# YooSungHyun/RNNTransducer

Measured on AMD Instinct MI355X. Metric: utterances/sec, higher is better.
Workload: dtype f32

## Files before the change

### rnntransducer_amd/csrc/gemm_hp.hip

```cpp
#include "common.hpp"

#include <stdlib.h>

namespace rnnt {
namespace {

typedef _Float16 f16x8 __attribute__((ext_vector_type(8)));
typedef __attribute__((address_space(3))) void lds_void;

constexpr int HP_BM = 256, HP_BN = 256, HP_BK = 32;
constexpr int HP_STAGE = (HP_BM + HP_BN) * 128;
constexpr int HP_RSRC = 0x00027000;

__device__ __forceinline__ float hp_scale_from_amax(unsigned amax_bits) {
  int eb = (int)((amax_bits >> 23) & 255u);
  if (eb == 0) return 1.0f;
  eb = eb < 15 ? 15 : eb;
  return __uint_as_float((unsigned)(268 - eb) << 23);
}
__device__ __forceinline__ float hp_inv_scale_from_amax(unsigned amax_bits) {
  int eb = (int)((amax_bits >> 23) & 255u);
  if (eb == 0) return 1.0f;
  eb = eb < 15 ? 15 : eb;
  return __uint_as_float((unsigned)(eb - 14) << 23);
}

__global__ void __launch_bounds__(256) hp_colmax_kernel(const float* __restrict__ x, long rows, int C, long ld, long rows_per_chunk,
                                                        unsigned* __restrict__ out) {
  const int c = blockIdx.x * 256 + threadIdx.x;
  if (c >= C) return;
  const long r0 = (long)blockIdx.y * rows_per_chunk, r1 = min(rows, r0 + rows_per_chunk);
  unsigned m = 0;
  for (long r = r0; r < r1; ++r) m = max(m, __float_as_uint(x[r * ld + c]) & 0x7fffffffu);
  if (m != 0) atomicMax(out + c, m);
}

__device__ __forceinline__ void hp_split8(const float (&x)[8], float scale, u32x4& hi, u32x4& lo) {
  f16x8 h, l;
#pragma unroll
  for (int e = 0; e < 8; ++e) {
    const float v = x[e] * scale;
    const _Float16 a = (_Float16)v;
    h[e] = a;
    l[e] = (_Float16)(v - (float)a);
  }
  hi = __builtin_bit_cast(u32x4, h);
  lo = __builtin_bit_cast(u32x4, l);
}

__global__ void __launch_bounds__(256) hp_split_kernel(const float* __restrict__ x, long rows, int K, long ld, unsigned* __restrict__ amax,
                                                       char* __restrict__ out, const int* __restrict__ rowidx) {
  const int Kp = (K + 31) & ~31, cpr = Kp >> 3;
  const int lane = threadIdx.x & 63;
  const bool vec = (ld & 3) == 0 && (reinterpret_cast<uintptr_t>(x) & 15) == 0;
  for (long ri = (long)blockIdx.x * 4 + (threadIdx.x >> 6); ri < rows; ri += (long)gridDim.x * 4) {
    const long r = rowidx ? (long)rowidx[ri] : ri;
    const float* row = x + r * ld;
    unsigned m = 0;
    for (int c = lane; c < cpr; c += 64) {
      const int k = 8 * c;
      if (vec && k + 7 < K) {
        const u32x4 a = *reinterpret_cast<const u32x4*>(row + k), b = *reinterpret_cast<const u32x4*>(row + k + 4);
#pragma unroll
        for (int e = 0; e < 4; ++e) m = max(m, max(a[e] & 0x7fffffffu, b[e] & 0x7fffffffu));
      } else {
#pragma unroll
        for (int e = 0; e < 8; ++e)
          if (k + e < K) m = max(m, __float_as_uint(row[k + e]) & 0x7fffffffu);
      }
    }
#pragma unroll
    for (int o = 32; o > 0; o >>= 1) m = max(m, (unsigned)__shfl_xor((int)m, o));
    if (lane == 0) amax[r] = m;
    const float scale = hp_scale_from_amax(m);
    for (int c = lane; c < cpr; c += 64) {
      const int k = 8 * c;
      float v[8];
      if (vec && k + 7 < K) {
        const f32x4 a = *reinterpret_cast<const f32x4*>(row + k), b = *reinterpret_cast<const f32x4*>(row + k + 4);
        v[0] = a[0]; v[1] = a[1]; v[2] = a[2]; v[3] = a[3]; v[4] = b[0]; v[5] = b[1]; v[6] = b[2]; v[7] = b[3];
      } else {
#pragma unroll
        for (int e = 0; e < 8; ++e) v[e] = (k + e < K) ? row[k + e] : 0.f;
      }
      u32x4 hi, lo;
      hp_split8(v, scale, hi, lo);
      char* dst = out + (r * (Kp >> 5) + (c >> 2)) * 128 + 16 * (c & 3);
      *reinterpret_cast<u32x4*>(dst) = hi;
      *reinterpret_cast<u32x4*>(dst + 64) = lo;
    }
  }
}

__global__ void __launch_bounds__(256) hp_split_t_kernel(const float* __restrict__ x, int R, int K, long ld, int Ksrc, int shift,
                                                         const unsigned* __restrict__ amax, char* __restrict__ out,
                                                         const int* __restrict__ kidx) {
  __shared__ float tile[32][257];
  const int kb = blockIdx.x, r0 = blockIdx.y * 256;
  const int tid = threadIdx.x;
  const bool vec = (ld & 3) == 0 && (reinterpret_cast<uintptr_t>(x) & 15) == 0;
#pragma unroll
  for (int q = 0; q < 8; ++q) {
    const int kk = 4 * q + (tid >> 6);
    const int kdst = kb * 32 + kk;
    const int ksrc = (kidx ? (kdst < K ? kidx[kdst] : 0) : kdst) + shift;
    const int c = 4 * (tid & 63);
    f32x4 v = {0.f, 0.f, 0.f, 0.f};
    if (kdst < K && ksrc >= 0 && ksrc < Ksrc) {
      const float* src = x + (long)ksrc * ld + r0 + c;
      if (vec && r0 + c + 3 < R) {
        v = *reinterpret_cast<const f32x4*>(src);
      } else {
#pragma unroll
        for (int e = 0; e < 4; ++e)
          if (r0 + c + e < R) v[e] = src[e];
      }
    }
#pragma unroll
    for (int e = 0; e < 4; ++e) tile[kk][c + e] = v[e];
  }
  __syncthreads();
  const int Kp32 = (K + 31) >> 5;
#pragma unroll
  for (int ps = 0; ps < 4; ++ps) {
    const int rl = (tid >> 2) + 64 * ps, ch = tid & 3;
    if (r0 + rl < R) {
      float v[8];
#pragma unroll
      for (int e = 0; e < 8; ++e) v[e] = tile[8 * ch + e][rl];
      u32x4 hi, lo;
      hp_split8(v, hp_scale_from_amax(amax[r0 + rl]), hi, lo);
      char* dst = out + ((long)(r0 + rl) * Kp32 + kb) * 128 + 16 * ch;
      *reinterpret_cast<u32x4*>(dst) = hi;
      *reinterpret_cast<u32x4*>(dst + 64) = lo;
    }
  }
}

__global__ void __launch_bounds__(256) hp_split_both_kernel(const float* __restrict__ x, int M, int C, long ld, const unsigned* __restrict__ rowmax,
                                                            const unsigned* __restrict__ colmax, char* __restrict__ out_rm, char* __restrict__ out_t,
                                                            const int* __restrict__ rowidx) {
  __shared__ float tile[32][257];
  const int kb = blockIdx.x, c0 = blockIdx.y * 256;
  const int tid = threadIdx.x;
  const int Cp = (C + 31) & ~31;
  const bool vec = (ld & 3) == 0 && (reinterpret_cast<uintptr_t>(x) & 15) == 0;
#pragma unroll
  for (int q = 0; q < 4; ++q) {
    const int row = 8 * q + (tid >> 5), col = 8 * (tid & 31);
    const int ri = kb * 32 + row, c = c0 + col;
    const int r = (rowidx && ri < M) ? rowidx[ri] : ri;
    float v[8] = {0.f, 0.f, 0.f, 0.f, 0.f, 0.f, 0.f, 0.f};
    if (ri < M && c < C) {
      const float* src = x + (long)r * ld + c;
      if (vec && c + 7 < C) {
        const f32x4 a = *reinterpret_cast<const f32x4*>(src), b = *reinterpret_cast<const f32x4*>(src + 4);
        v[0] = a[0]; v[1] = a[1]; v[2] = a[2]; v[3] = a[3]; v[4] = b[0]; v[5] = b[1]; v[6] = b[2]; v[7] = b[3];
      } else {
#pragma unroll
        for (int e = 0; e < 8; ++e)
          if (c + e < C) v[e] = src[e];
      }
    }
    if (ri < M && c < Cp) {
      u32x4 hi, lo;
      hp_split8(v, hp_scale_from_amax(rowmax[r]), hi, lo);
      char* dst = out_rm + ((long)r * (Cp >> 5) + (c >> 5)) * 128 + 16 * ((c >> 3) & 3);
      *reinterpret_cast<u32x4*>(dst) = hi;
      *reinterpret_cast<u32x4*>(dst + 64) = lo;
    }
#pragma unroll
    for (int e = 0; e < 8; ++e) tile[row][col + e] = v[e];
  }
  __syncthreads();
  const int Mp32 = (M + 31) >> 5;
#pragma unroll
  for (int ps = 0; ps < 4; ++ps) {
    const int rl = (tid >> 2) + 64 * ps, ch = tid & 3;
    if (c0 + rl < C) {
      float v[8];
#pragma unroll
      for (int e = 0; e < 8; ++e) v[e] = tile[8 * ch + e][rl];
      u32x4 hi, lo;
      hp_split8(v, hp_scale_from_amax(colmax[c0 + rl]), hi, lo);
      char* dst = out_t + ((long)(c0 + rl) * Mp32 + kb) * 128 + 16 * ch;
      *reinterpret_cast<u32x4*>(dst) = hi;
      *reinterpret_cast<u32x4*>(dst + 64) = lo;
    }
  }
}

struct HpGemmK {
  int M, N, nkt;
  const char* A; unsigned a_pitch, a_bytes;
  const char* B; unsigned b_pitch, b_bytes;
  const unsigned* a_amax; const unsigned* b_amax;
  float* C; int c_div; long c_so, c_si;
  const float* bias;
  unsigned flags;
  int splits, kt_per_split;
  float* slab;
  int tiles_m, tiles_n;
  int group_m;
  const int* a_rowidx;
  const int* c_rowidx;
};

// ... 153 lines not shown
  return n * tiles_m + m;
}

template <bool F16>
__global__ void __launch_bounds__(512, 1) gemm_hp_kernel(const HpGemmK p) {
  extern __shared__ __attribute__((aligned(16))) char lds[];
  int bid = hp_xcd_remap(blockIdx.x, p.tiles_m * p.tiles_n);
  if (p.group_m > 0) bid = hp_grouped_tile(bid, p.tiles_m, p.tiles_n, p.group_m);
  hp_tile256<F16>(p, bid, blockIdx.y, lds);
}

constexpr int HPQ_MAX = 4;
struct HpGemmQ {
  HpGemmK prob[HPQ_MAX];
  int unit_end[HPQ_MAX];
  int nprob;
  unsigned xcd_skip;
  unsigned* counter;
};

template <bool F16>
__global__ void __launch_bounds__(512, 1) gemm_hpq_kernel(const HpGemmQ q) {
  extern __shared__ __attribute__((aligned(16))) char lds[];
  unsigned xcc;
  asm volatile("s_getreg_b32 %0, hwreg(HW_REG_XCC_ID)" : "=s"(xcc));
  xcc &= 7u;
  if ((q.xcd_skip >> xcc) & 1u) return;
  const unsigned allow = ~q.xcd_skip & 0xffu;
  const int nq = __builtin_popcount(allow);
  const int mine = __builtin_popcount(allow & ((1u << xcc) - 1u));
  int* next = reinterpret_cast<int*>(lds + 2 * HP_STAGE);
  const int total = q.unit_end[q.nprob - 1];
  for (int hop = 0; hop < nq; ++hop) {
    const int qi = (mine + hop) % nq;
    const int lo = (int)((long)total * qi / nq), hi = (int)((long)total * (qi + 1) / nq);
    while (true) {
      if (threadIdx.x == 0) {
        const int got = lo + (int)atomicAdd(q.counter + qi, 1u);
        *next = got;
        if (got < hi) atomicAdd(q.counter + 8, 1u);
      }
      __syncthreads();
      const int u = __builtin_amdgcn_readfirstlane(*next);
      __syncthreads();
      if (u >= hi) break;
      int pi = 0;
      while (u >= q.unit_end[pi]) ++pi;
      const HpGemmK& p = q.prob[pi];
      const int local = u - (pi ? q.unit_end[pi - 1] : 0);
      const int tn = local % p.tiles_n, z = (local / p.tiles_n) % p.splits, tm = local / (p.tiles_n * p.splits);
      hp_tile256<F16>(p, tn * p.tiles_m + tm, z, lds);
    }
  }
}

__global__ void hpq_check_kernel(unsigned* counter, unsigned total, unsigned* status) {
  if (counter[8] != total) {
    counter[9] = 1u;
    if (status) __hip_atomic_store(status, 2u, __ATOMIC_RELAXED, __HIP_MEMORY_SCOPE_AGENT);
  }
}

__global__ void __launch_bounds__(256) hp_splitk_reduce_kernel(const HpGemmK p) {
  const long total = (long)p.M * p.N;
  for (long i = (long)blockIdx.x * 256 + threadIdx.x; i < total; i += (long)gridDim.x * 256) {
    const int m = (int)(i / p.N), n = (int)(i % p.N);
    float s = 0.f;
    for (int z = 0; z < p.splits; ++z) s += p.slab[(long)z * total + i];
    if (p.bias) s += p.bias[n];
    const int mo = p.c_rowidx ? p.c_rowidx[m] : m;
    const long off = (long)(mo / p.c_div) * p.c_so + (long)(mo % p.c_div) * p.c_si + n;
    if (p.flags & RNNT_GEMM_ACCUM) s += p.C[off];
    p.C[off] = s;
  }
}

}

size_t hp_plane_bytes(int64_t rows, int64_t K) { return (size_t)rows * (size_t)ceil_div(K, 32) * 128; }

int hp_colmax(const float* x, int64_t rows, int64_t C, int64_t ld, uint32_t* amax, hipStream_t s) {
  RNNT_CHECK_HIP(hipMemsetAsync(amax, 0, (size_t)C * 4, s));
  if (rows == 0 || C == 0) return RNNT_OK;
  long chunks = ceil_div(2048, ceil_div(C, 256));
  if (chunks > ceil_div(rows, 64)) chunks = ceil_div(rows, 64);
  if (chunks < 1) chunks = 1;
  const long rpc = ceil_div(rows, chunks);
  ProfScope prof(RNNT_K_HP_SPLIT, 4.0 * (double)rows * (double)C, s);
  hipLaunchKernelGGL(hp_colmax_kernel, dim3((unsigned)ceil_div(C, 256), (unsigned)ceil_div(rows, rpc)), dim3(256), 0, s, x, (long)rows, (int)C,
                     (long)ld, rpc, amax);
  RNNT_CHECK_LAUNCH();
  return RNNT_OK;
}

int hp_split(const float* x, int64_t rows, int64_t K, int64_t ld, uint32_t* amax, void* planes, hipStream_t s, const int* rowidx) {
  if (rows == 0) return RNNT_OK;
  const long blocks = ceil_div(rows, 4);
  ProfScope prof(RNNT_K_HP_SPLIT, 8.0 * (double)rows * (double)K, s);
  hipLaunchKernelGGL(hp_split_kernel, dim3((unsigned)(blocks < 8192 ? blocks : 8192)), dim3(256), 0, s, x, (long)rows, (int)K, (long)ld, amax,
                     (char*)planes, rowidx);
  RNNT_CHECK_LAUNCH();
  return RNNT_OK;
}

int hp_split_t(const float* x, int64_t R, int64_t K, int64_t ld, int64_t Ksrc, int64_t shift, const uint32_t* amax, void* planes,
               hipStream_t s, const int* kidx) {
  if (R == 0 || K == 0) return RNNT_OK;
  ProfScope prof(RNNT_K_HP_SPLIT, 8.0 * (double)R * (double)K, s);
  hipLaunchKernelGGL(hp_split_t_kernel, dim3((unsigned)ceil_div(K, 32), (unsigned)ceil_div(R, 256)), dim3(256), 0, s, x, (int)R, (int)K, (long)ld,
                     (int)Ksrc, (int)shift, amax, (char*)planes, kidx);
  RNNT_CHECK_LAUNCH();
  return RNNT_OK;
}

int hp_split_both(const float* x, int64_t M, int64_t C, int64_t ld, const uint32_t* rowmax, const uint32_t* colmax, void* planes_rm,
                  void* planes_t, hipStream_t s, const int* rowidx) {
  if (M == 0 || C == 0) return RNNT_OK;
  ProfScope prof(RNNT_K_HP_SPLIT, 12.0 * (double)M * (double)C, s);
  hipLaunchKernelGGL(hp_split_both_kernel, dim3((unsigned)ceil_div(M, 32), (unsigned)ceil_div(C, 256)), dim3(256), 0, s, x, (int)M, (int)C, (long)ld,
                     rowmax, colmax, (char*)planes_rm, (char*)planes_t, rowidx);
  RNNT_CHECK_LAUNCH();
  return RNNT_OK;
}

struct HpGemmPlan {
  int tiles_m, tiles_n, group_m, splits, kt_per_split;
  size_t workspace_bytes_wanted;
};
static HpGemmPlan hp_gemm_plan(int64_t M, int64_t N, int64_t K, size_t workspace_bytes) {
  HpGemmPlan pl;
  pl.tiles_m = (int)ceil_div(M, HP_BM); pl.tiles_n = (int)ceil_div(N, HP_BN);
  const long tiles = (long)pl.tiles_m * pl.tiles_n;
  const long nkt = ceil_div(K, HP_BK);
  {
    static const int env_gm = getenv("RNNT_GEMM_HP_GROUP_M") ? atoi(getenv("RNNT_GEMM_HP_GROUP_M")) : -1;
    pl.group_m = env_gm >= 0 ? env_gm : (tiles >= 256 ? 8 : 4);
  }
  long want = 1;
  if (tiles < 192 && nkt >= 64) {
    want = ceil_div(256, tiles);
    if (want > nkt / 32) want = nkt / 32;
    if (want > 32) want = 32;
    if (want < 2) want = 1;
  }
  const size_t slab = (size_t)M * (size_t)N * 4;
  pl.workspace_bytes_wanted = want >= 2 ? (size_t)want * slab : 0;
  const size_t by_ws = workspace_bytes / slab;
  long splits = (size_t)want > by_ws ? (long)by_ws : want;
  if (splits < 2) splits = 1;
  pl.kt_per_split = (int)ceil_div(nkt, splits);
  pl.splits = (int)ceil_div(nkt, pl.kt_per_split);
  return pl;
}

size_t hp_gemm_workspace_bytes(int64_t M, int64_t N, int64_t K) { return hp_gemm_plan(M, N, K, 0).workspace_bytes_wanted; }

int hp_gemm(const void* A, const uint32_t* a_amax, const void* B, const uint32_t* b_amax, int64_t M, int64_t N, int64_t K, float* C,
            int64_t c_div, int64_t c_so, int64_t c_si, const float* bias, unsigned flags, void* workspace, size_t workspace_bytes,
            hipStream_t s, const int* a_rowidx, int64_t a_plane_rows, const int* c_rowidx) {
  RNNT_CHECK_ARG(A && B && C && a_amax && b_amax, "gemm_hp: null operand");
  RNNT_CHECK_ARG(!a_rowidx || a_plane_rows >= M, "gemm_hp: a gathered A operand needs the row count of its planes");
  RNNT_CHECK_ARG(M >= 1 && N >= 1 && K >= 1 && M < (1ll << 31) && N < (1ll << 31) && K < (1ll << 31), "gemm_hp: bad dims");
  RNNT_CHECK_ARG(c_div >= 1, "gemm_hp: c_div must be >= 1");
  RNNT_CHECK_ARG(((reinterpret_cast<uintptr_t>(A) | reinterpret_cast<uintptr_t>(B)) & 127) == 0, "gemm_hp: planes must be 128-byte aligned");
  HpGemmK k;
  k.M = (int)M; k.N = (int)N; k.nkt = (int)ceil_div(K, HP_BK);
  const size_t ab = hp_plane_bytes(a_rowidx ? a_plane_rows : M, K), bb = hp_plane_bytes(N, K);
  RNNT_CHECK_ARG(ab < (1ull << 32) && bb < (1ull << 32), "gemm_hp: an operand exceeds the 4 GB a buffer resource addresses");
  k.A = (const char*)A; k.a_pitch = (unsigned)k.nkt * 128u; k.a_bytes = (unsigned)ab;
  k.B = (const char*)B; k.b_pitch = (unsigned)k.nkt * 128u; k.b_bytes = (unsigned)bb;
  k.a_amax = a_amax; k.b_amax = b_amax;
  k.C = C; k.c_div = (int)(c_div > 0x7fffffff ? 0x7fffffff : c_div); k.c_so = c_so; k.c_si = c_si;
  k.bias = bias; k.flags = flags;
  k.a_rowidx = a_rowidx; k.c_rowidx = c_rowidx;
  const bool f16 = (flags & RNNT_GEMM_HP_F16) != 0u;
  const HpGemmPlan pl = hp_gemm_plan(M, N, K, workspace ? workspace_bytes : 0);
  k.tiles_m = pl.tiles_m; k.tiles_n = pl.tiles_n; k.group_m = pl.group_m;
  k.splits = pl.splits; k.kt_per_split = pl.kt_per_split;
  const int tiles = k.tiles_m * k.tiles_n, splits = k.splits;
  k.slab = (float*)workspace;
  if (f16) RNNT_CHECK_HIP(hipFuncSetAttribute((const void*)gemm_hp_kernel<true>, hipFuncAttributeMaxDynamicSharedMemorySize, 2 * HP_STAGE));
  else RNNT_CHECK_HIP(hipFuncSetAttribute((const void*)gemm_hp_kernel<false>, hipFuncAttributeMaxDynamicSharedMemorySize, 2 * HP_STAGE));
  {
    ProfScope prof(RNNT_K_GEMM_HP, 2.0 * (double)M * (double)N * (double)K, s);
    if (f16) hipLaunchKernelGGL(gemm_hp_kernel<true>, dim3(tiles, splits), dim3(512), 2 * HP_STAGE, s, k);
    else hipLaunchKernelGGL(gemm_hp_kernel<false>, dim3(tiles, splits), dim3(512), 2 * HP_STAGE, s, k);
    RNNT_CHECK_LAUNCH();
    if (splits > 1) {
      const long blocks = ceil_div((long)M * N, 256);
      hipLaunchKernelGGL(hp_splitk_reduce_kernel, dim3((unsigned)(blocks < 2048 ? blocks : 2048)), dim3(256), 0, s, k);
      RNNT_CHECK_LAUNCH();
    }
  }
// ... 190 lines not shown
```

### rnntransducer_amd/csrc/lstm_layer.hip

```cpp
#include "lstm_shared.hpp"

#include <string.h>

namespace rnnt {
namespace {

__global__ void db_reduce_kernel(const float* __restrict__ part, int rows_per_dir, int H, int ngate, float* __restrict__ o0,
                                 float* __restrict__ o1, int accumulate, float* __restrict__ p0 = nullptr,
                                 float* __restrict__ p1 = nullptr) {
  const int c = blockIdx.x * 256 + threadIdx.x, d = blockIdx.y;
  if (c >= 4 * H || (c & 3) >= ngate) return;
  const float* src = part + (long)d * rows_per_dir * 4 * H + c;
  float s = 0.f;
  for (int r = 0; r < rows_per_dir; ++r) s += src[(long)r * 4 * H];
  float* o = (d ? o1 : o0) + (c & 3) * H + (c >> 2);
  *o = accumulate ? *o + s : s;
  float* q = d ? p1 : p0;
  if (q) {
    q += (c & 3) * H + (c >> 2);
    *q = accumulate ? *q + s : s;
  }
}
__global__ void permute_w_kernel(const float* __restrict__ w0, const float* __restrict__ w1, int H, int I, int ngate,
                                 float* __restrict__ out) {
  const long per = (long)4 * H * I;
  const long idx = (long)blockIdx.x * 256 + threadIdx.x;
  const int d = blockIdx.y;
  if (idx >= per) return;
  const int k = (int)(idx % I), r = (int)(idx / I);
  const float* w = d ? w1 : w0;
  out[d * per + idx] = (r & 3) < ngate ? w[(long)((r & 3) * H + (r >> 2)) * I + k] : 0.f;
}
__global__ void __launch_bounds__(256) zero_padded_rows_kernel(float* __restrict__ x, const int* __restrict__ lens, int T, int B, int I) {
  const int lane = threadIdx.x & 63;
  const long nrow = (long)T * B;
  const long nw = ((long)gridDim.x * blockDim.x) >> 6;
  for (long r = ((long)blockIdx.x * blockDim.x + threadIdx.x) >> 6; r < nrow; r += nw) {
    if ((int)(r / B) < lens[r % B]) continue;
    float* row = x + r * I;
    for (int i = lane; i < I; i += 64) row[i] = 0.f;
  }
}
__global__ void unpermute_w_kernel(const float* __restrict__ in, int H, int I, long in_dir_stride, int ngate,
                                   float* __restrict__ o0, float* __restrict__ o1, int accumulate, float* __restrict__ p0 = nullptr,
                                   float* __restrict__ p1 = nullptr) {
  const long per = (long)4 * H * I;
  const long idx = (long)blockIdx.x * 256 + threadIdx.x;
  const int d = blockIdx.y;
  if (idx >= per) return;
  const int k = (int)(idx % I), r = (int)(idx / I);
  float* o = d ? o1 : o0;
  if ((r & 3) < ngate) {
    const long off = (long)((r & 3) * H + (r >> 2)) * I + k;
    const float v = in[d * in_dir_stride + idx];
    o[off] = accumulate ? o[off] + v : v;
    float* q = d ? p1 : p0;
    if (q) q[off] = accumulate ? q[off] + v : v;
  }
}
__global__ void permute_bias_kernel(const float* __restrict__ bi0, const float* __restrict__ bh0,
                                    const float* __restrict__ bi1, const float* __restrict__ bh1, int H, int ngate,
                                    int gru, float* __restrict__ out) {
  const int idx = blockIdx.x * 256 + threadIdx.x;
  const int d = blockIdx.y;
  if (idx >= 4 * H) return;
  const int g = idx & 3, src = g * H + (idx >> 2);
  float v = 0.f;
  if (g < ngate) {
    const float bi = d ? bi1[src] : bi0[src], bh = d ? bh1[src] : bh0[src];
    v = (gru && g == 2) ? bi : bi + bh;
  }
  out[d * 4 * H + idx] = v;
}

inline bool use_hp(int T, int B, int I, int H, int D) {
  if (getenv("RNNT_GEMM_NO_HP")) return false;
  const long M = (long)T * B, N4 = (long)D * 4 * H;
  const long Iw = I > D * H ? I : (long)D * H;
  const size_t lim = (size_t)1 << 32;
  if (hp_plane_bytes(M, Iw) >= lim || hp_plane_bytes(Iw, M) >= lim || hp_plane_bytes(M, N4) >= lim || hp_plane_bytes(N4, M) >= lim ||
      hp_plane_bytes(H, M) >= lim)
    return false;
  return M >= 1024 && N4 >= 512 && H >= 128 && (getenv("RNNT_GEMM_FORCE_HP") || (M * N4 >= (1l << 22)));
}

enum class Form { NONE, V1, V2, V34, V5 };

struct LayerPlan {
  bool accepted;
  Form form;
  Plan v1;
  Plan2 p2;
  bool hp;
  bool takes_row_idx;
  bool takes_f16;
  int recurrence_xcds;
  int cus;
  size_t nflags, hx_bytes;
};

inline int cus_or_mi355x() {
  const int cus = device_cus();
  return cus > 0 ? cus : 256;
}

LayerPlan resolve_plan(int T, int B, int I, int H, int D, int cell, int cus) {
  LayerPlan lp = {};
  lp.form = Form::NONE;
  lp.recurrence_xcds = 8;
  lp.cus = cus;
  if (T < 1 || B < 1 || I < 1 || H < 4 || D < 1 || D > 2) return lp;
  lp.accepted = make_plan(B, H, D, cus, &lp.v1);
  Plan2 v2, v34;
  const bool has2 = make_plan2(B, H, D, cus, &v2), has34 = make_plan3(B, H, D, cus, &v34);
// ... 127 lines not shown
  RNNT_CHECK_ARG(d->cell >= RNNT_CELL_LSTM && d->cell <= RNNT_CELL_RNN_RELU, "lstm: unknown cell type %d", d->cell);
  RNNT_CHECK_ARG(d->lens && d->x && d->y && d->gates && (d->cst || d->cell != RNNT_CELL_LSTM), "lstm: null tensor");
  for (int k = 0; k < d->D; ++k)
    RNNT_CHECK_ARG(d->w_ih[k] && d->w_hh[k] && d->b_ih[k] && d->b_hh[k], "lstm: null weight (direction %d)", k);
  RNNT_CHECK_ARG(d->dropout_p >= 0.f && d->dropout_p < 1.f, "lstm: dropout_p must be in [0,1)");
  RNNT_CHECK_ARG(d->dropout_p == 0.f || d->y_drop, "lstm: dropout_p > 0 needs y_drop");
  RNNT_CHECK_ARG(d->x_abs_bound >= 0.f && d->x_abs_bound < 1e30f, "lstm: x_abs_bound must be 0 (measure) or a finite positive bound");
  RNNT_CHECK_ARG(!d->row_idx || (d->n_rows >= 1 && d->n_rows <= (int64_t)d->T * d->B), "lstm: row_idx needs 1 <= n_rows <= T*B (got %d)", d->n_rows);
  *w = carve_lstm(d->workspace, d->T, d->B, d->I, d->H, d->D, *lp);
  RNNT_CHECK_ARG(d->workspace && d->workspace_bytes >= w->total, "lstm: workspace too small (%zu < %zu)",
                 d->workspace_bytes, w->total);
  RNNT_CHECK_ARG((reinterpret_cast<uintptr_t>(d->gates) & 15) == 0 && (reinterpret_cast<uintptr_t>(d->y) & 15) == 0 &&
                     (reinterpret_cast<uintptr_t>(d->cst) & 15) == 0 && (reinterpret_cast<uintptr_t>(d->aux) & 15) == 0 &&
                     (reinterpret_cast<uintptr_t>(d->workspace) & 255) == 0,
                 "lstm: gates/y/cst must be 16-byte aligned, workspace 256-byte aligned");
  return RNNT_OK;
}

template <class P>
P second(P const (&x)[2], int D) { return D > 1 ? x[1] : x[0]; }

inline int gate_count(int cell) { return cell == RNNT_CELL_LSTM ? 4 : (cell == RNNT_CELL_GRU ? 3 : 1); }

inline bool x_is_plain(const rnnt_lstm_desc* d) { return d->x_sb == d->I && d->x_st == (int64_t)d->B * d->I; }

inline bool ragged_call(const rnnt_lstm_desc* d, const LayerPlan& lp) {
  return d->row_idx && d->n_rows > 0 && d->n_rows < (int64_t)d->T * d->B && x_is_plain(d) && lp.takes_row_idx;
}

void fill_kernel_args(const rnnt_lstm_desc* d, const LayerPlan& lp, const LstmWs& w, LstmK* k) {
  k->T = d->T; k->B = d->B; k->H = d->H; k->D = d->D;
  k->Bp = lp.v1.Bp; k->LDW = lp.v1.LDW;
  if (lp.form == Form::V2 || lp.form == Form::V34 || lp.form == Form::V5) {
    k->NC = lp.p2.NC; k->Hs = lp.p2.HS; k->G = lp.p2.G; k->Bg = lp.p2.Bg; k->Kp = lp.p2.Kp;
  } else {
    k->NC = lp.v1.NC; k->Hs = lp.v1.Hs; k->G = 1; k->Bg = d->B; k->Kp = d->H;
  }
  k->lens = d->lens; k->gates = d->gates; k->cst = d->cst; k->y = d->y;
  k->ydrop = d->dropout_p > 0.f ? d->y_drop : nullptr;
  k->keep_scale = d->dropout_p > 0.f ? 1.f / (1.f - d->dropout_p) : 1.f;
  k->drop_thresh = (unsigned)((double)d->dropout_p * 4294967296.0);
  k->seed = d->dropout_seed;
  k->w_hh[0] = d->w_hh[0]; k->w_hh[1] = second(d->w_hh, d->D);
  k->hx = w.hx; k->status = d->status ? d->status : w.flags; k->flags = w.flags + 16;
  k->dy = nullptr;
  k->cell = d->cell;
  k->b_hh[0] = d->b_hh[0]; k->b_hh[1] = second(d->b_hh, d->D);
  k->aux = d->aux;
  k->NGL = d->D;
  k->dbp = w.dbp; k->dbhp = w.dbp + w.dbp_half;
  k->dbg = getenv("RNNT_LSTM_DBG") ? w.dbg : nullptr;
  k->xcc = w.flags + 16 + w.nflags;
  k->allow_local = getenv("RNNT_LSTM_NO_XCD_LOCAL") ? 0 : 1;
  k->hw_math = getenv("RNNT_LSTM_EXACT_MATH") ? 0 : 1;
  k->pause = 0;
  k->gbound = 0;
  k->colmax = k->colmax_h = nullptr;
  k->rowmax = nullptr;
}

int launch_recurrence(const LayerPlan& lp, const LstmK& k, bool backward, bool f16, hipStream_t s) {
  switch (lp.form) {
    case Form::V5:
      return backward ? lstm5_bwd_launch(k, lp.p2, k.cell, s, f16) : lstm5_fwd_launch(k, lp.p2, k.cell, s, f16);
    case Form::V34:
      return backward ? lstm4_bwd_launch(k, lp.p2, k.cell, s) : lstm3_fwd_launch(k, lp.p2, k.cell, s);
    case Form::V2:
      return backward ? lstm2_bwd_launch(k, lp.p2, k.cell, s) : lstm2_fwd_launch(k, lp.p2, k.cell, s);
    case Form::V1:
      return backward ? lstm1_bwd_launch(k, lp.v1, s) : lstm1_fwd_launch(k, lp.v1, s);
    case Form::NONE:
      break;
  }
  if (backward) set_error("rnn: GRU / Elman cells need the grouped decomposition; B=%d H=%d does not fit", k.B, k.H);
  else set_error("rnn: GRU / Elman cells need the grouped decomposition (B/G <= 16 rows per group); B=%d H=%d does not fit", k.B, k.H);
  return RNNT_ERR_UNSUPPORTED;
}

int reset_exchange(const LstmWs& w, hipStream_t s) {
  RNNT_CHECK_HIP(hipMemsetAsync(w.flags, 0, (size_t)(reinterpret_cast<char*>(w.hx) - reinterpret_cast<char*>(w.flags)) + w.hx_bytes, s));
  return RNNT_OK;
}

int permute_w_ih(const rnnt_lstm_desc* d, const LstmWs& w, hipStream_t s) {
  const long per = (long)4 * d->H * d->I;
  hipLaunchKernelGGL(permute_w_kernel, dim3((unsigned)ceil_div(per, 256), d->D), dim3(256), 0, s, d->w_ih[0], second(d->w_ih, d->D),
                     d->H, d->I, gate_count(d->cell), w.wp);
  RNNT_CHECK_LAUNCH();
  return RNNT_OK;
}

int unpermute(const float* in, int H, int I, int D, int ngate, float* const (&out)[2], int acc, hipStream_t s, float* twin0 = nullptr,
              float* twin1 = nullptr) {
  const long per = (long)4 * H * I;
  hipLaunchKernelGGL(unpermute_w_kernel, dim3((unsigned)ceil_div(per, 256), D), dim3(256), 0, s, in, H, I, per, ngate, out[0],
                     second(out, D), acc, twin0, twin1);
  RNNT_CHECK_LAUNCH();
  return RNNT_OK;
}

}
}

using namespace rnnt;


extern "C" int32_t rnnt_hip_lstm_max_batch(int32_t H, int32_t D, int32_t cell) {
  const int cus = cus_or_mi355x();
  for (int B = 64; B >= 1; --B)
    if (resolve_plan(1, B, 1, H, D, cell, cus).form != Form::NONE) return B;
  return 0;
}

extern "C" int32_t rnnt_hip_lstm_takes_row_idx(int32_t T, int32_t B, int32_t I, int32_t H, int32_t D, int32_t cell) {
  return resolve_plan(T, B, I, H, D, cell, cus_or_mi355x()).takes_row_idx ? 1 : 0;
}

extern "C" int32_t rnnt_hip_lstm_takes_f16(int32_t T, int32_t B, int32_t I, int32_t H, int32_t D, int32_t cell) {
  return resolve_plan(T, B, I, H, D, cell, cus_or_mi355x()).takes_f16 ? 1 : 0;
}

extern "C" int32_t rnnt_hip_lstm_free_xcds(int32_t T, int32_t B, int32_t H, int32_t D, int32_t cell) {
  return 8 - resolve_plan(T, B, 1, H, D, cell, cus_or_mi355x()).recurrence_xcds;
}

extern "C" size_t rnnt_hip_lstm_workspace_bytes(int32_t T, int32_t B, int32_t I, int32_t H, int32_t D) {
  const LayerPlan lp = resolve_plan(T, B, I, H, D, RNNT_CELL_LSTM, cus_or_mi355x());
  return lp.accepted ? carve_lstm(nullptr, T, B, I, H, D, lp).total : 0;
}

static int lstm_fwd_impl(const rnnt_lstm_desc* d, uint32_t precision, void* stream) {
  LayerPlan lp;
  LstmWs w;
  if (int rc = check_desc(d, &lp, &w)) return rc;
  hipStream_t s = (hipStream_t)stream;
  const int H = d->H, D = d->D, I = d->I;
  const int64_t M = (int64_t)d->T * d->B, N4 = (int64_t)D * 4 * H;
  const bool f16 = precision == RNNT_PRECISION_F16 && lp.takes_f16;
  const unsigned hpf = f16 ? RNNT_GEMM_HP_F16 : 0u;
  const bool ragged = ragged_call(d, lp);
  const bool hp_proj = w.hp && x_is_plain(d) && I >= 32;

  if (int rc = permute_w_ih(d, w, s)) return rc;
  hipLaunchKernelGGL(permute_bias_kernel, dim3((unsigned)ceil_div(4 * H, 256), D), dim3(256), 0, s, d->b_ih[0], d->b_hh[0],
                     second(d->b_ih, D), second(d->b_hh, D), H, gate_count(d->cell), d->cell == RNNT_CELL_GRU ? 1 : 0, w.bp);
  RNNT_CHECK_LAUNCH();
  if (hp_proj) {
    const int64_t Mv = ragged ? d->n_rows : M;
    const int* ridx = ragged ? d->row_idx : nullptr;
    if (int rc = hp_split(d->x, Mv, I, I, w.amax_x, w.hp_x, s, ridx)) return rc;
    if (int rc = hp_split(w.wp, N4, I, I, w.amax_w, w.hp_w, s)) return rc;
    if (int rc = hp_gemm(w.hp_x, w.amax_x, w.hp_w, w.amax_w, Mv, N4, I, d->gates, 1, N4, 0, w.bp, hpf, nullptr, 0, s, ridx, M, ridx)) return rc;
  } else {
    rnnt_gemm_desc g = {};
    g.M = M; g.N = N4; g.K = I;
    g.A = d->x; g.a_div = d->B; g.a_so = d->x_st; g.a_si = d->x_sb; g.a_sk = 1; g.a_mc = 0;
    g.B = w.wp; g.b_sn = I; g.b_sk = 1;
    g.C = d->gates; g.c_div = 1; g.c_so = g.N; g.c_si = 0;
    g.bias = w.bp;
    if (int rc = rnnt_hip_gemm_f32(&g, s)) return rc;
  }
  if (int rc = reset_exchange(w, s)) return rc;
  LstmK k;
  fill_kernel_args(d, lp, w, &k);
  k.gbound = ragged ? 1 : 0;
  return launch_recurrence(lp, k, false, f16, s);
}

extern "C" int rnnt_hip_lstm_fwd(const rnnt_lstm_desc* d, void* stream) { return lstm_fwd_impl(d, RNNT_PRECISION_FP32, stream); }

extern "C" int rnnt_hip_lstm_fwd_ex(const rnnt_lstm_desc* d, uint32_t precision, void* stream) {
  RNNT_CHECK_ARG(precision == RNNT_PRECISION_FP32 || precision == RNNT_PRECISION_F16, "lstm_fwd_ex: precision must be 0 (fp32) or 1 (f16), got %u",
                 precision);
  return lstm_fwd_impl(d, precision, stream);
}

static int lstm_bwd_impl(const rnnt_lstm_bwd_desc* bd, uint32_t precision, void* stream) {
  RNNT_CHECK_ARG(bd != nullptr, "lstm_bwd: null descriptor");
  const rnnt_lstm_desc* d = &bd->f;
  LayerPlan lp;
  LstmWs w;
  if (int rc = check_desc(d, &lp, &w)) return rc;
  RNNT_CHECK_ARG(bd->dy, "lstm_bwd: null dy");
  const int T = d->T, B = d->B, H = d->H, D = d->D, I = d->I;
  const bool gru = d->cell == RNNT_CELL_GRU;
  const int ngate = gate_count(d->cell);
  RNNT_CHECK_ARG(!gru || d->aux, "lstm_bwd: GRU needs the aux buffer (T,B,D*4H)");
  for (int k = 0; k < D; ++k) RNNT_CHECK_ARG(!gru || bd->db_hh[k], "lstm_bwd: GRU needs db_hh");
  const int acc = bd->accumulate ? 1 : 0;
  float* twin0 = gru ? nullptr : bd->db_hh[0];
  float* twin1 = gru ? nullptr : second(bd->db_hh, D);
  if (twin0 == bd->db[0]) twin0 = nullptr;
  if (twin1 == second(bd->db, D)) twin1 = nullptr;
  const float* ghid = gru ? d->aux : d->gates;
  RNNT_CHECK_ARG(x_is_plain(d), "lstm_bwd: x must be time-major contiguous (T,B,I)");
  for (int k = 0; k < D; ++k) RNNT_CHECK_ARG(bd->dw_ih[k] && bd->dw_hh[k] && bd->db[k], "lstm_bwd: null gradient output");
  hipStream_t s = (hipStream_t)stream;
  RNNT_CHECK_ARG(bd->phase >= RNNT_LSTM_BWD_ALL && bd->phase <= RNNT_LSTM_BWD_WEIGHTS, "lstm_bwd: phase must be 0, 1 or 2");
  const bool do_recur = bd->phase != RNNT_LSTM_BWD_WEIGHTS, do_weights = bd->phase != RNNT_LSTM_BWD_RECUR;

  const bool f16 = precision == RNNT_PRECISION_F16 && lp.takes_f16;
  const unsigned hpf = f16 ? RNNT_GEMM_HP_F16 : 0u;
  const bool ragged = ragged_call(d, lp);
  const int* ridx = ragged ? d->row_idx : nullptr;
  const int64_t M = (int64_t)T * B, N4 = (int64_t)D * 4 * H;
  const int64_t Mv = ragged ? d->n_rows : M;
  const bool hp_in = w.hp && I >= 128;
  const bool hp_dwih = hp_in || (w.hp && I >= 32 && !getenv("RNNT_GEMM_HP_NO_NARROW"));
  const bool fused_db = lp.form == Form::V34 || lp.form == Form::V5;
  const int db_rows = lp.p2.G * 4 * lp.p2.BQ;
  const bool v5_maxima = lp.form == Form::V5 && w.hp;
  const bool both = v5_maxima && !gru && hp_in && bd->dx && !getenv("RNNT_GEMM_HP_NO_FUSED_SPLIT");
  const unsigned xcd_skip =
      (lp.form == Form::V5 && bd->beside_recurrence && lp.recurrence_xcds <= 4 && lp.cus == 256) ? (1u << lp.recurrence_xcds) - 1u : 0u;
  const bool grouped = hp_in && T > 1 && !gru && (xcd_skip != 0u || getenv("RNNT_GEMM_HP_GROUP")) && !getenv("RNNT_GEMM_HP_NO_GROUP");
  int rc = RNNT_OK;

  if (do_recur)
    if ((rc = reset_exchange(w, s))) return rc;
  LstmK k;
  fill_kernel_args(d, lp, w, &k);
  k.dy = bd->dy;
  k.gbound = ragged ? 1 : 0;
  if (v5_maxima) {
    k.colmax = w.amax_dg_cols;
    k.colmax_h = w.amax_dgh_cols;
    if (both) k.rowmax = w.amax_dg_rows;
    unsigned* first = both ? k.rowmax : k.colmax;
    if (do_recur) RNNT_CHECK_HIP(hipMemsetAsync(first, 0, (size_t)(w.amax_dgh_cols + N4 - first) * 4, s));
  }
  if (do_recur || lp.form == Form::NONE)
    if ((rc = launch_recurrence(lp, k, true, f16, s))) return rc;

  if (w.hp) {
    if (do_recur && hp_in && bd->dx) {
      if (both) rc = hp_split_both(d->gates, Mv, N4, N4, w.amax_dg_rows, w.amax_dg_cols, w.hp_dg, w.hp_dgt, s, ridx);
      else rc = hp_split(d->gates, Mv, N4, N4, w.amax_dg_rows, w.hp_dg, s, ridx);
      if (rc) return rc;
    }
    if (do_weights && !v5_maxima)
      if ((rc = hp_colmax(d->gates, M, N4, N4, w.amax_dg_cols, s))) return rc;
    if (do_weights && !both)
      if ((rc = hp_split_t(d->gates, N4, Mv, N4, M, 0, w.amax_dg_cols, w.hp_dgt, s, ridx))) return rc;
  }
  if (do_recur && bd->dx) {
    if ((rc = permute_w_ih(d, w, s))) return rc;
    if (hp_in) {
      if ((rc = hp_colmax(w.wp, N4, I, I, w.amax_wt, s))) return rc;
      if ((rc = hp_split_t(w.wp, I, N4, I, N4, 0, w.amax_wt, w.hp_w, s))) return rc;
      if ((rc = hp_gemm(w.hp_dg, w.amax_dg_rows, w.hp_w, w.amax_wt, Mv, I, N4, bd->dx, 1, I, 0, nullptr, hpf, nullptr, 0, s, ridx, M, ridx))) return rc;
    } else {
      rnnt_gemm_desc g = {};
      g.M = M; g.N = I; g.K = N4;
      g.A = d->gates; g.a_div = 1; g.a_so = N4; g.a_si = 0; g.a_sk = 1; g.a_mc = 0;
      g.B = w.wp; g.b_sn = 1; g.b_sk = I;
      g.C = bd->dx; g.c_div = 1; g.c_so = I; g.c_si = 0;
      if ((rc = rnnt_hip_gemm_f32(&g, s))) return rc;
    }
    if (ragged) {
      hipLaunchKernelGGL(zero_padded_rows_kernel, dim3((unsigned)(ceil_div(M, 4) < 2048 ? ceil_div(M, 4) : 2048)), dim3(256), 0, s, bd->dx, d->lens, T, B, I);
      RNNT_CHECK_LAUNCH();
    }
  }
  if (!do_weights) return RNNT_OK;
  if (hp_dwih) {
    if (d->x_abs_bound > 0.f) {
      uint32_t bits;
      memcpy(&bits, &d->x_abs_bound, 4);
      RNNT_CHECK_HIP(hipMemsetD32Async((hipDeviceptr_t)w.amax_xt, (int)bits, (size_t)I, s));
    } else if ((rc = hp_colmax(d->x, M, I, I, w.amax_xt, s))) return rc;
    if ((rc = hp_split_t(d->x, I, Mv, I, M, 0, w.amax_xt, w.hp_x, s, ridx))) return rc;
    if (!grouped)
      if ((rc = hp_gemm(w.hp_dgt, w.amax_dg_cols, w.hp_x, w.amax_xt, N4, I, Mv, w.wp, 1, I, 0, nullptr, hpf, w.scratch, w.scratch_bytes, s))) return rc;
  } else {
    rnnt_gemm_desc g = {};
    g.M = N4; g.N = I; g.K = M;
    g.A = d->gates; g.a_mc = 1; g.a_sk = N4; g.a_div = 1;
    g.B = d->x; g.b_sn = 1; g.b_sk = I;
    g.C = w.wp; g.c_div = 1; g.c_so = I; g.c_si = 0;
    g.workspace = w.scratch; g.workspace_bytes = w.scratch_bytes;
    if ((rc = rnnt_hip_gemm_f32(&g, s))) return rc;
  }
  if (!grouped)
    if ((rc = unpermute(w.wp, H, I, D, ngate, bd->dw_ih, acc, s))) return rc;
  if (w.hp && T > 1) {
    if (d->cell != RNNT_CELL_RNN_RELU) {
      RNNT_CHECK_HIP(hipMemsetD32Async((hipDeviceptr_t)w.amax_yt, 0x3f800000, (size_t)D * H, s));
    } else if ((rc = hp_colmax(d->y, M, (int64_t)D * H, (int64_t)D * H, w.amax_yt, s))) return rc;
    uint32_t* a_dgh = w.amax_dg_cols;
    if (gru) {
      if (v5_maxima) a_dgh = w.amax_dgh_cols;
      else if ((rc = hp_colmax(ghid, M, N4, N4, a_dgh, s))) return rc;
      if ((rc = hp_split_t(ghid, N4, Mv, N4, M, 0, a_dgh, w.hp_dgt, s, ridx))) return rc;
    }
    HpProblem pr[HP_GROUP_MAX];
    int npr = 0;
    if (grouped) pr[npr++] = HpProblem{w.hp_dgt, w.amax_dg_cols, w.hp_x, w.amax_xt, N4, I, Mv, w.wp, I, hpf};
    for (int dir = 0; dir < D; ++dir) {
      char* yt = w.hp_yt + (size_t)dir * hp_plane_bytes(H, M);
      uint32_t* a_y = w.amax_yt + (int64_t)dir * H;
      float* dwhh = w.dwhh + (int64_t)dir * 4 * H * H;
      if ((rc = hp_split_t(d->y + (int64_t)dir * H, H, Mv, (int64_t)D * H, M, dir == 0 ? -B : B, a_y, yt, s, ridx))) return rc;
      const char* ag = w.hp_dgt + (size_t)dir * 4 * H * (size_t)ceil_div(Mv, 32) * 128;
      if (grouped) {
        pr[npr++] = HpProblem{ag, a_dgh + (int64_t)dir * 4 * H, yt, a_y, 4 * H, H, Mv, dwhh, H, hpf};
        continue;
      }
      if ((rc = hp_gemm(ag, a_dgh + (int64_t)dir * 4 * H, yt, a_y, 4 * H, H, Mv, dwhh, 1, H, 0, nullptr, hpf, w.scratch, w.scratch_bytes, s)))
        return rc;
    }
    if (grouped) {
      if ((rc = hp_gemm_grouped(pr, npr, xcd_skip, reinterpret_cast<unsigned*>(w.scratch), (char*)w.scratch + HPQ_HEADER_BYTES,
                                w.scratch_bytes - HPQ_HEADER_BYTES, s, k.status)))
        return rc;
      if ((rc = unpermute(w.wp, H, I, D, ngate, bd->dw_ih, acc, s))) return rc;
    }
  } else
  for (int dir = 0; dir < D; ++dir) {
    rnnt_gemm_desc g = {};
    g.M = 4 * H; g.N = H; g.K = (int64_t)(T - 1) * B;
    const int64_t shift_g = dir == 0 ? (int64_t)B * N4 : 0;
    const int64_t shift_y = dir == 0 ? 0 : (int64_t)B * D * H;
    g.A = ghid + shift_g + (int64_t)dir * 4 * H; g.a_mc = 1; g.a_sk = N4; g.a_div = 1;
    g.B = d->y + shift_y + (int64_t)dir * H; g.b_sn = 1; g.b_sk = (int64_t)D * H;
    g.C = w.dwhh + (int64_t)dir * 4 * H * H; g.c_div = 1; g.c_so = H; g.c_si = 0;
    g.workspace = w.scratch; g.workspace_bytes = w.scratch_bytes;
    if (g.K > 0) {
      if ((rc = rnnt_hip_gemm_f32(&g, s))) return rc;
    } else {
      RNNT_CHECK_HIP(hipMemsetAsync(g.C, 0, (size_t)4 * H * H * 4, s));
    }
// ... 53 lines not shown
```

Before: 1297.

## Fuse weight column-max into permute kernel and retile colmax and transposed split

The column-max reduction over the permuted input weights now happens inside the permute kernel through atomicMax, which removes a separate hp_colmax pass over the weight matrix. The permute kernel is reorganised as 2D blocks, each thread covering 16 rows of one column. hp_colmax is rewritten to read four columns per thread with 16-byte loads, reduce across lanes with shuffles and LDS, and pick its grid shape from C. The transposed split tiles 64 columns instead of 256 to give small R more blocks. The memset of amax_wt is skipped when v5_maxima is set, which could leave stale maxima if that path relied on hp_colmax clearing the buffer.

```diff
diff --git a/rnntransducer_amd/csrc/gemm_hp.hip b/rnntransducer_amd/csrc/gemm_hp.hip
--- a/rnntransducer_amd/csrc/gemm_hp.hip
+++ b/rnntransducer_amd/csrc/gemm_hp.hip
@@ -11,6 +11,7 @@
 constexpr int HP_BM = 256, HP_BN = 256, HP_BK = 32;
 constexpr int HP_STAGE = (HP_BM + HP_BN) * 128;
 constexpr int HP_RSRC = 0x00027000;
+constexpr int HPT_COLS = 64;
 
 __device__ __forceinline__ float hp_scale_from_amax(unsigned amax_bits) {
   int eb = (int)((amax_bits >> 23) & 255u);
@@ -26,13 +27,49 @@
 }
 
 __global__ void __launch_bounds__(256) hp_colmax_kernel(const float* __restrict__ x, long rows, int C, long ld, long rows_per_chunk,
-                                                        unsigned* __restrict__ out) {
-  const int c = blockIdx.x * 256 + threadIdx.x;
-  if (c >= C) return;
+                                                        int tx_log2, unsigned* __restrict__ out) {
+  __shared__ unsigned red[4][256];
+  const int TX = 1 << tx_log2, RY = 256 >> tx_log2;
+  const int tid = threadIdx.x, lane = tid & 63, wave = tid >> 6;
+  const int g = tid & (TX - 1), ry = tid >> tx_log2;
+  const int c0 = blockIdx.x * TX * 4, c = c0 + g * 4;
   const long r0 = (long)blockIdx.y * rows_per_chunk, r1 = min(rows, r0 + rows_per_chunk);
-  unsigned m = 0;
-  for (long r = r0; r < r1; ++r) m = max(m, __float_as_uint(x[r * ld + c]) & 0x7fffffffu);
-  if (m != 0) atomicMax(out + c, m);
+  const bool vec = (ld & 3) == 0 && (reinterpret_cast<uintptr_t>(x) & 15) == 0 && c + 3 < C;
+  unsigned m[4] = {0u, 0u, 0u, 0u};
+  if (vec) {
+    const float* p = x + c;
+    long r = r0 + ry;
+    for (; r + 7 * RY < r1; r += 8 * RY) {
+      u32x4 v[8];
+#pragma unroll
+      for (int i = 0; i < 8; ++i) v[i] = *reinterpret_cast<const u32x4*>(p + (r + i * RY) * ld);
+#pragma unroll
+      for (int i = 0; i < 8; ++i)
+#pragma unroll
+        for (int e = 0; e < 4; ++e) m[e] = max(m[e], v[i][e] & 0x7fffffffu);
+    }
+    for (; r < r1; r += RY) {
+      const u32x4 a = *reinterpret_cast<const u32x4*>(p + r * ld);
+#pragma unroll
+      for (int e = 0; e < 4; ++e) m[e] = max(m[e], a[e] & 0x7fffffffu);
+    }
+  } else if (c < C) {
+    for (long r = r0 + ry; r < r1; r += RY)
+#pragma unroll
+      for (int e = 0; e < 4; ++e)
+        if (c + e < C) m[e] = max(m[e], __float_as_uint(x[r * ld + c + e]) & 0x7fffffffu);
+  }
+  for (int o = TX; o < 64; o <<= 1)
+#pragma unroll
+    for (int e = 0; e < 4; ++e) m[e] = max(m[e], (unsigned)__shfl_xor((int)m[e], o));
+  if (lane < TX)
+#pragma unroll
+    for (int e = 0; e < 4; ++e) red[wave][4 * lane + e] = m[e];
+  __syncthreads();
+  if (tid < 4 * TX && c0 + tid < C) {
+    const unsigned v = max(max(red[0][tid], red[1][tid]), max(red[2][tid], red[3][tid]));
+    if (v != 0) atomicMax(out + c0 + tid, v);
+  }
 }
 
 __device__ __forceinline__ void hp_split8(const float (&x)[8], float scale, u32x4& hi, u32x4& lo) {
@@ -95,16 +132,18 @@
 __global__ void __launch_bounds__(256) hp_split_t_kernel(const float* __restrict__ x, int R, int K, long ld, int Ksrc, int shift,
                                                          const unsigned* __restrict__ amax, char* __restrict__ out,
                                                          const int* __restrict__ kidx) {
-  __shared__ float tile[32][257];
-  const int kb = blockIdx.x, r0 = blockIdx.y * 256;
+  constexpr int TPR = HPT_COLS / 4;
+  constexpr int RPP = 256 / TPR;
+  __shared__ float tile[32][HPT_COLS + 1];
+  const int kb = blockIdx.x, r0 = blockIdx.y * HPT_COLS;
   const int tid = threadIdx.x;
   const bool vec = (ld & 3) == 0 && (reinterpret_cast<uintptr_t>(x) & 15) == 0;
-#pragma unroll
-  for (int q = 0; q < 8; ++q) {
-    const int kk = 4 * q + (tid >> 6);
+  const int c = 4 * (tid % TPR);
+#pragma unroll
+  for (int q = 0; q < 32 / RPP; ++q) {
+    const int kk = RPP * q + tid / TPR;
     const int kdst = kb * 32 + kk;
     const int ksrc = (kidx ? (kdst < K ? kidx[kdst] : 0) : kdst) + shift;
-    const int c = 4 * (tid & 63);
     f32x4 v = {0.f, 0.f, 0.f, 0.f};
     if (kdst < K && ksrc >= 0 && ksrc < Ksrc) {
       const float* src = x + (long)ksrc * ld + r0 + c;
@@ -122,7 +161,7 @@
   __syncthreads();
   const int Kp32 = (K + 31) >> 5;
 #pragma unroll
-  for (int ps = 0; ps < 4; ++ps) {
+  for (int ps = 0; ps < HPT_COLS / 64; ++ps) {
     const int rl = (tid >> 2) + 64 * ps, ch = tid & 3;
     if (r0 + rl < R) {
       float v[8];
@@ -442,13 +481,16 @@
 int hp_colmax(const float* x, int64_t rows, int64_t C, int64_t ld, uint32_t* amax, hipStream_t s) {
   RNNT_CHECK_HIP(hipMemsetAsync(amax, 0, (size_t)C * 4, s));
   if (rows == 0 || C == 0) return RNNT_OK;
-  long chunks = ceil_div(2048, ceil_div(C, 256));
-  if (chunks > ceil_div(rows, 64)) chunks = ceil_div(rows, 64);
+  int tx_log2 = 0;
+  while (tx_log2 < 6 && (4l << tx_log2) < C) ++tx_log2;
+  const long gx = ceil_div(C, 4l << tx_log2);
+  long chunks = ceil_div(512, gx);
+  if (chunks > ceil_div(rows, 128)) chunks = ceil_div(rows, 128);
   if (chunks < 1) chunks = 1;
   const long rpc = ceil_div(rows, chunks);
   ProfScope prof(RNNT_K_HP_SPLIT, 4.0 * (double)rows * (double)C, s);
-  hipLaunchKernelGGL(hp_colmax_kernel, dim3((unsigned)ceil_div(C, 256), (unsigned)ceil_div(rows, rpc)), dim3(256), 0, s, x, (long)rows, (int)C,
-                     (long)ld, rpc, amax);
+  hipLaunchKernelGGL(hp_colmax_kernel, dim3((unsigned)gx, (unsigned)ceil_div(rows, rpc)), dim3(256), 0, s, x, (long)rows, (int)C,
+                     (long)ld, rpc, tx_log2, amax);
   RNNT_CHECK_LAUNCH();
   return RNNT_OK;
 }
@@ -467,8 +509,9 @@
                hipStream_t s, const int* kidx) {
   if (R == 0 || K == 0) return RNNT_OK;
   ProfScope prof(RNNT_K_HP_SPLIT, 8.0 * (double)R * (double)K, s);
-  hipLaunchKernelGGL(hp_split_t_kernel, dim3((unsigned)ceil_div(K, 32), (unsigned)ceil_div(R, 256)), dim3(256), 0, s, x, (int)R, (int)K, (long)ld,
-                     (int)Ksrc, (int)shift, amax, (char*)planes, kidx);
+  RNNT_CHECK_ARG(ceil_div(R, HPT_COLS) <= 65535, "hp_split: more than %d rows in a transposed split", 65535 * HPT_COLS);
+  hipLaunchKernelGGL(hp_split_t_kernel, dim3((unsigned)ceil_div(K, 32), (unsigned)ceil_div(R, HPT_COLS)), dim3(256), 0, s, x, (int)R, (int)K,
+                     (long)ld, (int)Ksrc, (int)shift, amax, (char*)planes, kidx);
   RNNT_CHECK_LAUNCH();
   return RNNT_OK;
 }
diff --git a/rnntransducer_amd/csrc/lstm_layer.hip b/rnntransducer_amd/csrc/lstm_layer.hip
--- a/rnntransducer_amd/csrc/lstm_layer.hip
+++ b/rnntransducer_amd/csrc/lstm_layer.hip
@@ -21,15 +21,23 @@
     *q = accumulate ? *q + s : s;
   }
 }
-__global__ void permute_w_kernel(const float* __restrict__ w0, const float* __restrict__ w1, int H, int I, int ngate,
-                                 float* __restrict__ out) {
-  const long per = (long)4 * H * I;
-  const long idx = (long)blockIdx.x * 256 + threadIdx.x;
-  const int d = blockIdx.y;
-  if (idx >= per) return;
-  const int k = (int)(idx % I), r = (int)(idx / I);
+constexpr int PERMUTE_ROWS = 16;
+__global__ void __launch_bounds__(256) permute_w_kernel(const float* __restrict__ w0, const float* __restrict__ w1, int H, int I, int ngate,
+                                                        float* __restrict__ out, unsigned* __restrict__ colmax) {
+  const int k = blockIdx.x * blockDim.x + threadIdx.x;
+  const int d = blockIdx.z;
+  if (k >= I) return;
   const float* w = d ? w1 : w0;
-  out[d * per + idx] = (r & 3) < ngate ? w[(long)((r & 3) * H + (r >> 2)) * I + k] : 0.f;
+  float* o = out + (long)d * 4 * H * I + k;
+  const int r0 = (blockIdx.y * blockDim.y + threadIdx.y) * PERMUTE_ROWS, r1 = min(4 * H, r0 + PERMUTE_ROWS);
+  unsigned m = 0;
+#pragma unroll 8
+  for (int r = r0; r < r1; ++r) {
+    const float v = (r & 3) < ngate ? w[(long)((r & 3) * H + (r >> 2)) * I + k] : 0.f;
+    o[(long)r * I] = v;
+    m = max(m, __float_as_uint(v) & 0x7fffffffu);
+  }
+  if (colmax && m != 0) atomicMax(colmax + k, m);
 }
 __global__ void __launch_bounds__(256) zero_padded_rows_kernel(float* __restrict__ x, const int* __restrict__ lens, int T, int B, int I) {
   const int lane = threadIdx.x & 63;
@@ -323,10 +331,12 @@
   return RNNT_OK;
 }
 
-int permute_w_ih(const rnnt_lstm_desc* d, const LstmWs& w, hipStream_t s) {
-  const long per = (long)4 * d->H * d->I;
-  hipLaunchKernelGGL(permute_w_kernel, dim3((unsigned)ceil_div(per, 256), d->D), dim3(256), 0, s, d->w_ih[0], second(d->w_ih, d->D),
-                     d->H, d->I, gate_count(d->cell), w.wp);
+int permute_w_ih(const rnnt_lstm_desc* d, const LstmWs& w, hipStream_t s, uint32_t* colmax = nullptr) {
+  int tx = 256;
+  while (tx > 1 && tx / 2 >= d->I) tx /= 2;
+  const int ty = 256 / tx;
+  hipLaunchKernelGGL(permute_w_kernel, dim3((unsigned)ceil_div(d->I, tx), (unsigned)ceil_div(4 * d->H, ty * PERMUTE_ROWS), d->D), dim3(tx, ty), 0, s,
+                     d->w_ih[0], second(d->w_ih, d->D), d->H, d->I, gate_count(d->cell), w.wp, colmax);
   RNNT_CHECK_LAUNCH();
   return RNNT_OK;
 }
@@ -485,9 +495,9 @@
       if ((rc = hp_split_t(d->gates, N4, Mv, N4, M, 0, w.amax_dg_cols, w.hp_dgt, s, ridx))) return rc;
   }
   if (do_recur && bd->dx) {
-    if ((rc = permute_w_ih(d, w, s))) return rc;
+    if (hp_in && !v5_maxima) RNNT_CHECK_HIP(hipMemsetAsync(w.amax_wt, 0, (size_t)I * 4, s));
+    if ((rc = permute_w_ih(d, w, s, hp_in ? w.amax_wt : nullptr))) return rc;
     if (hp_in) {
-      if ((rc = hp_colmax(w.wp, N4, I, I, w.amax_wt, s))) return rc;
       if ((rc = hp_split_t(w.wp, I, N4, I, N4, 0, w.amax_wt, w.hp_w, s))) return rc;
       if ((rc = hp_gemm(w.hp_dg, w.amax_dg_rows, w.hp_w, w.amax_wt, Mv, I, N4, bd->dx, 1, I, 0, nullptr, hpf, nullptr, 0, s, ridx, M, ridx))) return rc;
     } else {
```

After: 1307, median of 6. About the same (+0.8%).
